# gk969/stm32-speech-recognition

Measured on AMD Instinct MI355X. Metric: utterances/sec (256-frame, 100 templates), higher is better.
Workload: dtype int32

## Files before the change

### stm32_speech_recognition_amd/csrc/k_mfcc.hip

```cpp
#include "sr_fft_dev.h"

#include <type_traits>

#ifndef SR_MEL_CHUNKED
#define SR_MEL_CHUNKED 1
#endif

namespace sr {

constexpr int kMfccWaves = 4;
constexpr int kFramesPerWave = 16, kFramesPerWaveMid = 4, kFramesPerWaveSmall = 1;
#ifndef SR_MAG_TAB_BINS
#define SR_MAG_TAB_BINS 8
#endif
constexpr int mfcc_tab_bins(int fpw) { return fpw == kFramesPerWave ? SR_MAG_TAB_BINS : 0; }
static_assert(SR_MAG_TAB_BINS == 0 || SR_MAG_TAB_BINS == 4 || SR_MAG_TAB_BINS == 8, "table bins per lane");
#ifndef SR_MFCC_PIPE
#define SR_MFCC_PIPE 1
#endif
#ifndef SR_MFCC_PIPE_PEEL
#define SR_MFCC_PIPE_PEEL 1
#endif
#ifndef SR_MFCC_PIPE_VMCNT
#define SR_MFCC_PIPE_VMCNT (SR_MFCC_PIPE_PEEL ? 3 : 0)
#endif
static_assert(SR_MFCC_PIPE_VMCNT == 0 || (SR_MFCC_PIPE_VMCNT == 3 && SR_MFCC_PIPE_PEEL), "younger loads counted by the wait");
constexpr bool mfcc_pipelined(int fpw) { return SR_MFCC_PIPE && mfcc_tab_bins(fpw) == 8; }
constexpr int kMelPad = kMel + 1;
__device__ __forceinline__ constexpr int mel_chunk_word(int j) { return 256 * ((j >> 2) & 1) + 4 * ((j >> 3) ^ (4 * ((j >> 2) & 1))) + (j & 3); }
constexpr int mfcc_wave_lds_words(int fpw) { return kXchgWords + fpw * kMelPad + 64; }

template <typename Base>
struct MfccTabArgs : Base {
    const uint16_t *mag_q;
    uint32_t mag_table_off;
};
template <typename Base>
constexpr int mfcc_feat_kind<MfccTabArgs<Base>> = mfcc_feat_kind<Base>;
template <typename Base>
static MfccTabArgs<Base> mfcc_tab_args(const Base &b, const MfccMagTab &tab)
{
    MfccTabArgs<Base> r;
    static_cast<Base &>(r) = b;
    r.mag_q = tab.mag_q;
    r.mag_table_off = tab.mag_table_off;
    return r;
}

template <int kFPW, typename Args = MfccTabArgs<MfccArgs>>
__global__ void __launch_bounds__(64 * kMfccWaves, 4) k_mfcc(const Args a)
{
    constexpr int kFeat = mfcc_feat_kind<Args>;
    constexpr uint32_t kFeatW = (kFeat == SR_FEAT_FFT || kFeat == SR_FEAT_MAG) ? kBins : kMel;
    constexpr int kWaveLdsWords = mfcc_wave_lds_words(kFPW);
    constexpr int kTabBins = mfcc_tab_bins(kFPW);
    constexpr bool kPipe = mfcc_pipelined(kFPW);
    extern __shared__ __attribute__((aligned(16))) uint32_t smem[];
    __shared__ uint32_t s_dctM[kCoef * kMelPad];
    __shared__ int s_dctS[kCoef * kMelPad];
    __shared__ u32x4 s_tw3[kTw3Row * 4], s_tw5[8 * 64];
    __shared__ u32x4 s_tm[4 * 64];
    const int lane = threadIdx.x & 63, w = __builtin_amdgcn_readfirstlane(threadIdx.x >> 6);
    uint32_t *buf = smem + w * kWaveLdsWords;
    uint32_t *xw = buf;
    uint32_t *powb = buf + kXchgWords, *moff = powb + kFPW * kMelPad;

    for (int i = threadIdx.x; i < kCoef * kMel; i += blockDim.x) {
        const int c = a.t.dct[i], o = (i / kMel) * kMelPad + i % kMel;
        s_dctM[o] = (uint32_t)(((c < 0 ? -c : c) * 262144 + 99) / 100);
        s_dctS[o] = (c > 0) - (c < 0);
    }
    __syncthreads();

    LaneTw tw;
    load_lane_tw(a.t, lane, tw);
    real_leg_tw(tw);
    if (w == 0 && lane < 4) {
        const uint32_t *f = &tw.s3[0][0][0];
#pragma unroll
        for (int c = 0; c < 8; c++) s_tw3[lane * kTw3Row + c] = u32x4{f[4 * c], f[4 * c + 1], f[4 * c + 2], f[4 * c + 3]};
    }
    if (w == 1 % kMfccWaves) store_tw32(s_tw5, lane, tw.s5);
#ifndef SR_INJECT_LDS_RACE
    if (w == 2 % kMfccWaves) {
#pragma unroll
        for (int c = 0; c < 2; c++) {
            s_tm[64 * c + lane] = *(const u32x4 *)(a.t.tri_even_m + 8 * lane + 4 * c);
            s_tm[64 * (c + 2) + lane] = *(const u32x4 *)(a.t.tri_odd_m + 8 * lane + 4 * c);
        }
    }
#endif
    __syncthreads();
#ifdef SR_INJECT_LDS_RACE
    if (w == 2 % kMfccWaves) {
#if SR_INJECT_LDS_RACE >= 2
        __builtin_amdgcn_s_sleep(127);
#endif
#pragma unroll
        for (int c = 0; c < 2; c++) {
            s_tm[64 * c + lane] = *(const u32x4 *)(a.t.tri_even_m + 8 * lane + 4 * c);
            s_tm[64 * (c + 2) + lane] = *(const u32x4 *)(a.t.tri_odd_m + 8 * lane + 4 * c);
        }
    }
#endif
    int hamm_m[3];
#pragma unroll
    for (int k = 0; k < 3; k++) hamm_m[k] = (lane + 64 * k < kFrameLen) ? hamm_fused_multiplier(a.t.hamm[lane + 64 * k]) : 0;
    int f_lo = 0, p_hi = 0, p_lo = 0, x_hi = 0, x_lo = 0;
    if (lane < kMel) {
        const int h = lane;
        f_lo = (h == 0) ? 0 : (int)a.t.tri_cen[h - 1];
        const int f_hi = (h == kMel - 1) ? kBins : (int)a.t.tri_cen[h + 1];
        const int ih = f_hi - 1, il = f_lo ? f_lo - 1 : 0, half = (h & 1) ? kBins : 0;
#if SR_MEL_CHUNKED
        p_hi = half + mel_chunk_word(ih), x_hi = (ih >> 3) > 0 ? (ih >> 3) - 1 : 0;
        p_lo = half + mel_chunk_word(il), x_lo = (il >> 3) > 0 ? (il >> 3) - 1 : 0;
#else
        p_hi = half + ih, x_hi = (ih >> 3) > 0 ? (ih >> 3) - 1 : 0;
        p_lo = half + il, x_lo = (il >> 3) > 0 ? (il >> 3) - 1 : 0;
#endif
    }
    const uint64_t mag_p = (uint64_t)a.mag_q;
    const u32x4 mag_rs = {(uint32_t)mag_p, (uint32_t)(mag_p >> 32) | (2u << 16), kMagTabEntries, 0x00027000u};
    const uint32_t tw_off = 32u * (uint32_t)lane;
#if SR_MEL_CHUNKED
    const int e_base = mel_chunk_word(lane);
    constexpr int kEs = 32, kEh = 128;
    const int c0 = mel_chunk_word(8 * lane), c1 = mel_chunk_word(8 * lane + 4);
#else
    const int e_base = lane;
    constexpr int kEs = 64, kEh = 256;
    const int c0 = 8 * lane, c1 = 8 * lane + 4;
#endif

    uint32_t item = blockIdx.x;
    uint32_t nx_nfrm = 0;
    int nx_mid = 0, nx_seg0 = 0;
    if (item < a.n_items) {
        const sr_vad_rec *rec = a.vad + item / a.tiles;
        nx_nfrm = rec->frm_num;
        nx_mid = (int)rec->atap.mid_val;
        nx_seg0 = rec->seg[0];
    }
    for (; item < a.n_items; item += gridDim.x) {
        const uint32_t b = item / a.tiles, tile = item - b * a.tiles;
        const uint32_t nfrm = nx_nfrm;
        const int mid = nx_mid, seg0 = nx_seg0;
        if (item + gridDim.x < a.n_items) {
            const sr_vad_rec *rec = a.vad + (item + gridDim.x) / a.tiles;
            nx_nfrm = rec->frm_num;
            nx_mid = (int)rec->atap.mid_val;
            nx_seg0 = rec->seg[0];
        }
        const uint16_t *row = a.pcm + (uint64_t)b * a.pcm_stride;
        int16_t *out = a.mfcc + (uint64_t)b * a.max_frames * kCoef;
        const uint32_t f0 = tile * (kMfccWaves * kFPW) + w * kFPW;
        uint32_t *frow = nullptr;
        if constexpr (kFeat != 0) frow = a.feat + (uint64_t)b * a.max_frames * kFeatW;
        uint32_t nf = 0;
        if (f0 < nfrm) nf = (nfrm - f0 < (uint32_t)kFPW) ? nfrm - f0 : (uint32_t)kFPW;

        uint32_t s_pp[3] = {0, 0, 0};
        if (nf) {
            const uint16_t *x = row + seg0 + (int)kHop * (int)f0;
#pragma unroll
            for (int k = 0; k < 3; k++) {
                const int i = lane + 64 * k;
                if (i < kFrameLen) s_pp[k] = *(const u32_align2 *)(x + i - 1);
            }
        }
        if constexpr (!kPipe)
        for (uint32_t fi = 0; fi < nf; fi++) {
#pragma unroll
            for (int k = 0; k < 3; k++) {
                const int i = lane + 64 * k;
                if (i < kFrameLen) k == 0 ? window_store<0>(xw, i, s_pp[k], mid, hamm_m[k]) : window_store<1>(xw, i, s_pp[k], mid, hamm_m[k]);
            }
            if (fi + 1 < nf) {
                const uint16_t *x = row + seg0 + (int)kHop * (int)(f0 + fi + 1);
#pragma unroll
                for (int k = 0; k < 3; k++) {
                    const int i = lane + 64 * k;
                    if (i < kFrameLen) s_pp[k] = *(const u32_align2 *)(x + i - 1);
                }
            }
            wave_sync();
            uint32_t v[4][4], u[4][4];
            fft_front_real160(xw, lane, tw, s_tw3, v);
            fft_exchange(buf, lane, v, u);
#pragma unroll
            for (int e4 = 0; e4 < 4; e4++) fft_pass4_dbl(u, e4, tw);
            wave_sync();
            uint32_t k5[4][4][2];
            load_tw32(s_tw5, lane, k5);
            uint32_t nn[8];
#pragma unroll
            for (int e3 = 0; e3 < 4; e3++) {
                bfly_pk_dbl<true, false, 0>(u[e3][0], u[e3][1], u[e3][2], u[e3][3], k5[e3][0][0], k5[e3][0][1], k5[e3][1][0],
                                            k5[e3][1][1], k5[e3][2][0], k5[e3][2][1], k5[e3][3][0], k5[e3][3][1]);
                if constexpr (kFeat == SR_FEAT_FFT) {
                    uint32_t *fr = frow + (f0 + fi) * kFeatW + lane + 64 * e3;
                    fr[0] = u[e3][0];
                    fr[256] = u[e3][1];
                }
                nn[2 * e3] = (uint32_t)sdot2z(u[e3][0], u[e3][0]);
                nn[2 * e3 + 1] = (uint32_t)sdot2z(u[e3][1], u[e3][1]);
            }
            const uint32_t nmax = max(max(max(max(nn[0], nn[1]), nn[2]), max(max(nn[3], nn[4]), nn[5])), max(nn[6], nn[7]));
#ifdef SR_TESTING
            const bool quiet = __builtin_expect(__builtin_amdgcn_ballot_w64(nmax > kMagSmallMax) == 0 && !a.mag_table_off, 1);
#else
            const bool quiet = __builtin_expect(__builtin_amdgcn_ballot_w64(nmax > kMagSmallMax) == 0, 1);
#endif
            u32x4 tw_e[2], tw_o[2];
            bool cheap = true;
            if (!quiet) {
#pragma unroll
                for (int c = 0; c < 2; c++) {
                    tw_e[c] = *(const u32x4 *)((const char *)a.t.tri_even32 + tw_off + 16 * c);
                    tw_o[c] = *(const u32x4 *)((const char *)a.t.tri_odd32 + tw_off + 16 * c);
                }
                cheap = __builtin_amdgcn_ballot_w64(nmax > a.mag_cheap_max) == 0;
            } else {
                asm volatile("" : "=v"(tw_e[0]), "=v"(tw_e[1]), "=v"(tw_o[0]), "=v"(tw_o[1]));
            }
            uint32_t *eb = buf + e_base;
            if (kTabBins > 0 && quiet) {
                uint32_t tq[8];
#pragma unroll
                for (int e3 = 0; e3 < 4; e3++) {
                    if constexpr (kTabBins == 8)
                        asm volatile("buffer_load_ushort %0, %1, %2, 0 idxen" : "=v"(tq[2 * e3]) : "v"(nn[2 * e3]), "s"(mag_rs));
                    asm volatile("buffer_load_ushort %0, %1, %2, 0 idxen" : "=v"(tq[2 * e3 + 1]) : "v"(nn[2 * e3 + 1]), "s"(mag_rs));
                }
                uint32_t q0s[4];
                if constexpr (kTabBins == 4) {
#pragma unroll
                    for (int e3 = 0; e3 < 4; e3++) q0s[e3] = cvt_u32(__builtin_amdgcn_sqrtf((float)(int)nn[2 * e3]) * 10.0f) << 2;
                }
                if constexpr (kTabBins == 8)
                    asm volatile("s_waitcnt vmcnt(0)" : "+v"(tq[0]), "+v"(tq[1]), "+v"(tq[2]), "+v"(tq[3]), "+v"(tq[4]), "+v"(tq[5]), "+v"(tq[6]), "+v"(tq[7]));
                else
                    asm volatile("s_waitcnt vmcnt(0)" : "+v"(tq[1]), "+v"(tq[3]), "+v"(tq[5]), "+v"(tq[7]));
#pragma unroll
                for (int e3 = 0; e3 < 4; e3++) {
                    uint32_t q0, q1 = tq[2 * e3 + 1];
                    if constexpr (kTabBins == 8) q0 = tq[2 * e3];
                    else q0 = q0s[e3];
                    if constexpr (kFeat == SR_FEAT_MAG) {
                        uint32_t *fr = frow + (f0 + fi) * kFeatW + lane + 64 * e3;
                        fr[0] = q0 >> 2;
                        fr[256] = q1 >> 2;
                    }
                    eb[kEs * e3] = umul24(q0, q0);
                    eb[kEs * e3 + kEh] = umul24(q1, q1);
                }
            } else if (cheap) {
#pragma unroll
                for (int e3 = 0; e3 < 4; e3++) {
                    const f32x2 m = f32x2{__builtin_amdgcn_sqrtf((float)(int)nn[2 * e3]), __builtin_amdgcn_sqrtf((float)(int)nn[2 * e3 + 1])} *
                                    f32x2{10.0f, 10.0f};
                    const uint32_t m0 = cvt_u32(m.x), m1 = cvt_u32(m.y);
                    if constexpr (kFeat == SR_FEAT_MAG) {
                        uint32_t *fr = frow + (f0 + fi) * kFeatW + lane + 64 * e3;
                        fr[0] = m0;
                        fr[256] = m1;
                    }
                    eb[kEs * e3] = umul24(m0, m0);
                    eb[kEs * e3 + kEh] = umul24(m1, m1);
                }
            } else {
#pragma unroll
                for (int e3 = 0; e3 < 4; e3++) {
                    const f32x2 m = sqrt_rn_int2(f32x2{(float)(int)nn[2 * e3], (float)(int)nn[2 * e3 + 1]}) * f32x2{10.0f, 10.0f};
                    const uint32_t m0 = cvt_u32(m.x), m1 = cvt_u32(m.y);
                    if constexpr (kFeat == SR_FEAT_MAG) {
                        uint32_t *fr = frow + (f0 + fi) * kFeatW + lane + 64 * e3;
                        fr[0] = m0;
                        fr[256] = m1;
                    }
                    eb[kEs * e3] = umul24(m0, m0);
                    eb[kEs * e3 + kEh] = umul24(m1, m1);
                }
            }
            wave_sync();
            uint32_t pe[8], po[8], xe, xo;
            {
                const uint4 q0 = *(const uint4 *)(buf + c0), q1 = *(const uint4 *)(buf + c1);
                const uint32_t e[8] = {q0.x, q0.y, q0.z, q0.w, q1.x, q1.y, q1.z, q1.w};
                uint32_t se = 0, so = 0;
                if (quiet) {
#pragma unroll
                    for (int c = 0; c < 2; c++) {
                        const u32x4 me = s_tm[64 * c + lane], mo = s_tm[64 * (c + 2) + lane];
#pragma unroll
                        for (int k = 0; k < 4; k++) {
                            const uint32_t es = kTabBins > 0 ? e[4 * c + k] : e[4 * c + k] << 4;
                            se += mel_term_fused(es, me[k]);
                            so += mel_term_fused(es, mo[k]);
                            pe[4 * c + k] = se;
                            po[4 * c + k] = so;
                        }
                    }
                } else {
#pragma unroll
                    for (int c = 0; c < 2; c++) {
#pragma unroll
                        for (int k = 0; k < 4; k++) {
                            se += e[4 * c + k] * tw_e[c][k] / 100u;
                            so += e[4 * c + k] * tw_o[c][k] / 100u;
                            pe[4 * c + k] = se;
                            po[4 * c + k] = so;
                        }
                    }
                }
                xe = wave_scan_incl(se);
                xo = wave_scan_incl(so);
            }
            *(uint4 *)(buf + c0) = make_uint4(pe[0], pe[1], pe[2], pe[3]);
            *(uint4 *)(buf + c1) = make_uint4(pe[4], pe[5], pe[6], pe[7]);
            *(uint4 *)(buf + kBins + c0) = make_uint4(po[0], po[1], po[2], po[3]);
            *(uint4 *)(buf + kBins + c1) = make_uint4(po[4], po[5], po[6], po[7]);
            buf[2 * kBins + lane] = xe;
            moff[lane] = xo;
            wave_sync();
            if (lane < kMel) {
                const uint32_t *X = (lane & 1) ? moff : buf + 2 * kBins;
                const uint32_t hi = buf[p_hi] + X[x_hi], lo = f_lo ? buf[p_lo] + X[x_lo] : 0u;
                powb[fi * kMelPad + lane] = hi - lo;
                if constexpr (kFeat == SR_FEAT_MEL) frow[(f0 + fi) * kFeatW + lane] = hi - lo;
            }
            wave_sync();
        } else {
            uint32_t mq[8] = {0, 0, 0, 0, 0, 0, 0, 0};
            bool pq = true;
            auto window = [&]() {
#pragma unroll
                for (int k = 0; k < 3; k++) {
                    const int i = lane + 64 * k;
                    if (i < kFrameLen) k == 0 ? window_store<0>(xw, i, s_pp[k], mid, hamm_m[k]) : window_store<1>(xw, i, s_pp[k], mid, hamm_m[k]);
                }
            };
            auto request = [&](uint32_t f) {
                const uint16_t *x = row + seg0 + (int)kHop * (int)(f0 + f);
#pragma unroll
                for (int k = 0; k < 3; k++) {
                    const int i = lane + 64 * k;
                    if (i < kFrameLen) s_pp[k] = *(const u32_align2 *)(x + i - 1);
                }
            };
            auto middle = [&](uint32_t fi, uint32_t (&v)[4][4], bool more) {
                uint32_t u[4][4];
                fft_exchange(buf, lane, v, u);
#pragma unroll
                for (int e4 = 0; e4 < 4; e4++) fft_pass4_dbl(u, e4, tw);
                wave_sync();
                uint32_t k5[4][4][2];
                load_tw32(s_tw5, lane, k5);
                uint32_t nn[8];
#pragma unroll
                for (int e3 = 0; e3 < 4; e3++) {
                    bfly_pk_dbl<true, false, 0>(u[e3][0], u[e3][1], u[e3][2], u[e3][3], k5[e3][0][0], k5[e3][0][1], k5[e3][1][0],
                                                k5[e3][1][1], k5[e3][2][0], k5[e3][2][1], k5[e3][3][0], k5[e3][3][1]);
                    if constexpr (kFeat == SR_FEAT_FFT) {
                        uint32_t *fr = frow + (f0 + fi) * kFeatW + lane + 64 * e3;
                        fr[0] = u[e3][0];
                        fr[256] = u[e3][1];
                    }
                    nn[2 * e3] = (uint32_t)sdot2z(u[e3][0], u[e3][0]);
                    nn[2 * e3 + 1] = (uint32_t)sdot2z(u[e3][1], u[e3][1]);
                }
                const uint32_t nmax = max(max(max(max(nn[0], nn[1]), nn[2]), max(max(nn[3], nn[4]), nn[5])), max(nn[6], nn[7]));
                if (more) {
                    wave_sync();
                    window();
                }
#ifdef SR_TESTING
                const bool quiet = __builtin_expect(__builtin_amdgcn_ballot_w64(nmax > kMagSmallMax) == 0 && !a.mag_table_off, 1);
#else
                const bool quiet = __builtin_expect(__builtin_amdgcn_ballot_w64(nmax > kMagSmallMax) == 0, 1);
#endif
                if (quiet) {
#pragma unroll
                    for (int k = 0; k < 8; k++) asm volatile("buffer_load_ushort %0, %1, %2, 0 idxen" : "=v"(mq[k]) : "v"(nn[k]), "s"(mag_rs));
                } else if (__builtin_amdgcn_ballot_w64(nmax > a.mag_cheap_max) == 0) {
#pragma unroll
                    for (int e3 = 0; e3 < 4; e3++) {
                        const f32x2 m = f32x2{__builtin_amdgcn_sqrtf((float)(int)nn[2 * e3]), __builtin_amdgcn_sqrtf((float)(int)nn[2 * e3 + 1])} *
                                        f32x2{10.0f, 10.0f};
                        mq[2 * e3] = cvt_u32(m.x);
                        mq[2 * e3 + 1] = cvt_u32(m.y);
                    }
                } else {
#pragma unroll
                    for (int e3 = 0; e3 < 4; e3++) {
                        const f32x2 m = sqrt_rn_int2(f32x2{(float)(int)nn[2 * e3], (float)(int)nn[2 * e3 + 1]}) * f32x2{10.0f, 10.0f};
                        mq[2 * e3] = cvt_u32(m.x);
                        mq[2 * e3 + 1] = cvt_u32(m.y);
                    }
                }
                pq = quiet;
                if (fi + 2 < nf) request(fi + 2);
            };
            auto back_end = [&](uint32_t r, auto young) {
                wave_sync();
                auto energies = [&]() {
                    uint32_t *eb = buf + e_base;
#pragma unroll
                    for (int e3 = 0; e3 < 4; e3++) {
                        const uint32_t q0 = mq[2 * e3], q1 = mq[2 * e3 + 1];
                        if constexpr (kFeat == SR_FEAT_MAG) {
                            uint32_t *fr = frow + (f0 + r) * kFeatW + lane + 64 * e3;
                            const uint32_t sh = pq ? 2u : 0u;
                            fr[0] = q0 >> sh;
                            fr[256] = q1 >> sh;
                        }
                        eb[kEs * e3] = umul24(q0, q0);
                        eb[kEs * e3 + kEh] = umul24(q1, q1);
                    }
                    wave_sync();
                };
                uint32_t pe[8], po[8], se = 0, so = 0;
                if (pq) {
                    if constexpr (decltype(young)::value)
                        asm volatile("s_waitcnt vmcnt(3)" : "+v"(mq[0]), "+v"(mq[1]), "+v"(mq[2]), "+v"(mq[3]), "+v"(mq[4]), "+v"(mq[5]), "+v"(mq[6]), "+v"(mq[7]));
                    else
                        asm volatile("s_waitcnt vmcnt(0)" : "+v"(mq[0]), "+v"(mq[1]), "+v"(mq[2]), "+v"(mq[3]), "+v"(mq[4]), "+v"(mq[5]), "+v"(mq[6]), "+v"(mq[7]));
                    energies();
                    const uint4 q0 = *(const uint4 *)(buf + c0), q1 = *(const uint4 *)(buf + c1);
                    const uint32_t e[8] = {q0.x, q0.y, q0.z, q0.w, q1.x, q1.y, q1.z, q1.w};
#pragma unroll
                    for (int c = 0; c < 2; c++) {
                        const u32x4 me = s_tm[64 * c + lane], mo = s_tm[64 * (c + 2) + lane];
#pragma unroll
                        for (int k = 0; k < 4; k++) {
                            se += mel_term_fused(e[4 * c + k], me[k]);
                            so += mel_term_fused(e[4 * c + k], mo[k]);
                            pe[4 * c + k] = se;
                            po[4 * c + k] = so;
                        }
                    }
                } else {
                    u32x4 tw_e[2], tw_o[2];
                    uint32_t off = tw_off;
                    asm("" : "+v"(off));
#pragma unroll
                    for (int c = 0; c < 2; c++) {
                        tw_e[c] = *(const u32x4 *)((const char *)a.t.tri_even32 + off + 16 * c);
                        tw_o[c] = *(const u32x4 *)((const char *)a.t.tri_odd32 + off + 16 * c);
                    }
                    energies();
                    const uint4 q0 = *(const uint4 *)(buf + c0), q1 = *(const uint4 *)(buf + c1);
                    const uint32_t e[8] = {q0.x, q0.y, q0.z, q0.w, q1.x, q1.y, q1.z, q1.w};
#pragma unroll
                    for (int c = 0; c < 2; c++) {
#pragma unroll
                        for (int k = 0; k < 4; k++) {
                            se += e[4 * c + k] * tw_e[c][k] / 100u;
                            so += e[4 * c + k] * tw_o[c][k] / 100u;
                            pe[4 * c + k] = se;
                            po[4 * c + k] = so;
                        }
                    }
                }
                const uint32_t xe = wave_scan_incl(se), xo = wave_scan_incl(so);
                *(uint4 *)(buf + c0) = make_uint4(pe[0], pe[1], pe[2], pe[3]);
                *(uint4 *)(buf + c1) = make_uint4(pe[4], pe[5], pe[6], pe[7]);
                *(uint4 *)(buf + kBins + c0) = make_uint4(po[0], po[1], po[2], po[3]);
                *(uint4 *)(buf + kBins + c1) = make_uint4(po[4], po[5], po[6], po[7]);
                buf[2 * kBins + lane] = xe;
                moff[lane] = xo;
                wave_sync();
                if (lane < kMel) {
                    const uint32_t *X = (lane & 1) ? moff : buf + 2 * kBins;
                    const uint32_t hi = buf[p_hi] + X[x_hi], lo = f_lo ? buf[p_lo] + X[x_lo] : 0u;
                    powb[r * kMelPad + lane] = hi - lo;
                    if constexpr (kFeat == SR_FEAT_MEL) frow[(f0 + r) * kFeatW + lane] = hi - lo;
                }
                wave_sync();
            };
            constexpr std::false_type kDrain{};
            if (nf) {
                window();
                if (nf > 1) request(1);
#if SR_MFCC_PIPE_PEEL
                constexpr std::integral_constant<bool, SR_MFCC_PIPE_VMCNT != 0> kSteady{};
                {
                    wave_sync();
                    uint32_t v[4][4];
                    fft_front_real160(xw, lane, tw, s_tw3, v);
                    middle(0, v, nf > 1);
                }
                for (uint32_t fi = 1; fi + 1 < nf; fi++) {
                    wave_sync();
                    uint32_t v[4][4];
                    fft_front_real160(xw, lane, tw, s_tw3, v);
                    back_end(fi - 1, kSteady);
                    middle(fi, v, true);
                }
                if (nf > 1) {
                    wave_sync();
                    uint32_t v[4][4];
                    fft_front_real160(xw, lane, tw, s_tw3, v);
                    back_end(nf - 2, kDrain);
                    middle(nf - 1, v, false);
                }
#else
                for (uint32_t fi = 0; fi < nf; fi++) {
                    wave_sync();
                    uint32_t v[4][4];
                    fft_front_real160(xw, lane, tw, s_tw3, v);
                    if (fi > 0) back_end(fi - 1, kDrain);
                    middle(fi, v, fi + 1 < nf);
                }
#endif
                back_end(nf - 1, kDrain);
            }
        }

        {
            constexpr int kLogRounds = (kFPW * kMelPad + 63) / 64;
            const uint32_t n_log = nf * kMelPad;
            uint32_t nv[kLogRounds], mv[kLogRounds];
            u32x2 tv[kLogRounds];
#pragma unroll
            for (int r = 0; r < kLogRounds; r++) {
                const uint32_t t = lane + 64u * r;
                nv[r] = powb[t];
                mv[r] = log100_est(nv[r]);
                tv[r] = *(const u32_pair_align4 *)((const char *)a.t.log_thr + 4u * mv[r]);
            }
#pragma unroll
            for (int r = 0; r < kLogRounds; r++) {
                const uint32_t t = lane + 64u * r;
                if (t < n_log) powb[t] = log100_fix(nv[r], mv[r], tv[r].x, tv[r].y) << 14;
            }
        }
        wave_sync();
        if constexpr (kFeat == SR_FEAT_LOGMEL) {
            uint32_t *fw = frow + f0 * kFeatW;
            for (uint32_t t = lane; t < nf * kFeatW; t += 64) {
                const uint32_t fi = t / kFeatW, h = t - fi * kFeatW;
                fw[t] = powb[fi * kMelPad + h] >> 14;
            }
        }
        {
            int16_t *out_w = out + (size_t)f0 * kCoef;
#pragma unroll
            for (uint32_t tl = lane; tl < (uint32_t)(kFPW * kCoef); tl += 64) {
                uint32_t t = tl;
                if constexpr (kPipe) asm volatile("" : "+v"(t));
                if (t < nf * kCoef) {
                    const uint32_t fi = umul24(t, 10923u) >> 17, h = t - umul24(fi, (uint32_t)kCoef);
                    const uint32_t *pw = powb + umul24(fi, (uint32_t)kMelPad), *dm = s_dctM + umul24(h, (uint32_t)kMelPad);
                    const int *ds = s_dctS + umul24(h, (uint32_t)kMelPad);
                    int acc = 0;
#pragma unroll
                    for (int i = 0; i < kMel; i++) acc = mad24((int)__umulhi(pw[i], dm[i]), ds[i], acc);
                    out_w[t] = (int16_t)acc;
                }
            }
        }
        wave_sync();
        {
            const uint32_t r0 = f0 + nf, r1 = (f0 + kFPW < a.max_frames) ? f0 + kFPW : a.max_frames;
            for (uint32_t t = r0 * kCoef + lane; t < r1 * kCoef && r0 < r1; t += 64) out[t] = 0;
        }
        if constexpr (kFeat != 0) {
            const uint32_t r0 = f0 + nf, r1 = (f0 + kFPW < a.max_frames) ? f0 + kFPW : a.max_frames;
            for (uint32_t t = r0 * kFeatW + lane; t < r1 * kFeatW && r0 < r1; t += 64) frow[t] = 0;
        }
    }
}

uint32_t mfcc_ext_frames_per_tile();
int mfcc_ext_occupancy(int *per_cu);
void launch_mfcc_ext(const MfccArgs &a, uint32_t grid, hipStream_t s);
void launch_mfcc_ext_features(const MfccArgs &a, int kind, uint32_t *feat, uint32_t grid, hipStream_t s);

uint32_t mfcc_frames_per_tile(uint32_t frame_len) { return frame_len == 320 ? mfcc_ext_frames_per_tile() : (uint32_t)(kMfccWaves * kFramesPerWave); }
uint32_t mfcc_frames_per_tile_small(uint32_t frame_len, uint32_t which)
{
    return frame_len == 320 ? mfcc_ext_frames_per_tile() : (uint32_t)(kMfccWaves * (which ? kFramesPerWaveSmall : kFramesPerWaveMid));
}

uint32_t mfcc_resident_workgroups(uint32_t frame_len)
{
    int dev = 0, n_cu = 0, per_cu = 0;
    if (hipGetDevice(&dev) != hipSuccess) return 0;
    if (hipDeviceGetAttribute(&n_cu, hipDeviceAttributeMultiprocessorCount, dev) != hipSuccess || n_cu < 1) return 0;
    int e;
    if (frame_len == 320)
        e = mfcc_ext_occupancy(&per_cu);
    else
        e = (int)hipOccupancyMaxActiveBlocksPerMultiprocessor(&per_cu, k_mfcc<kFramesPerWave>, 64 * kMfccWaves,
                                                              (size_t)kMfccWaves * mfcc_wave_lds_words(kFramesPerWave) * sizeof(uint32_t));
    if (e != (int)hipSuccess || per_cu < 1) return 0;
    return (uint32_t)(per_cu * n_cu);
}

void launch_mfcc(const MfccArgs &a, const MfccMagTab &tab, hipStream_t s)
{
    if (a.generic) {
        launch_mfcc_gen(a, s);
        return;
    }
    if (a.n_items == 0) return;
    const uint32_t cap = a.grid_cap ? a.grid_cap : 4096u;
    const uint32_t grid = a.n_items < cap ? a.n_items : cap;
    if (a.frame_len == 320) {
        launch_mfcc_ext(a, grid, s);
        return;
    }
    if (a.small_tiles == 2) {
        const size_t lds = (size_t)kMfccWaves * mfcc_wave_lds_words(kFramesPerWaveSmall) * sizeof(uint32_t);
        SR_LAUNCH_POINT(s, "k_mfcc");
        hipLaunchKernelGGL(k_mfcc<kFramesPerWaveSmall>, dim3(grid), dim3(64 * kMfccWaves), lds, s, mfcc_tab_args(a, tab));
        return;
    }
    if (a.small_tiles == 1) {
        const size_t lds = (size_t)kMfccWaves * mfcc_wave_lds_words(kFramesPerWaveMid) * sizeof(uint32_t);
        SR_LAUNCH_POINT(s, "k_mfcc");
        hipLaunchKernelGGL(k_mfcc<kFramesPerWaveMid>, dim3(grid), dim3(64 * kMfccWaves), lds, s, mfcc_tab_args(a, tab));
        return;
    }
    const size_t lds = (size_t)kMfccWaves * mfcc_wave_lds_words(kFramesPerWave) * sizeof(uint32_t);
    SR_LAUNCH_POINT(s, "k_mfcc");
    hipLaunchKernelGGL(k_mfcc<kFramesPerWave>, dim3(grid), dim3(64 * kMfccWaves), lds, s, mfcc_tab_args(a, tab));
}

template <int kFPW, int kKind>
static void launch_mfcc_feat_kind(const MfccArgs &a, const MfccMagTab &tab, uint32_t *feat, uint32_t grid, hipStream_t s)
{
    const size_t lds = (size_t)kMfccWaves * mfcc_wave_lds_words(kFPW) * sizeof(uint32_t);
    SR_LAUNCH_POINT(s, "k_mfcc");
    hipLaunchKernelGGL((k_mfcc<kFPW, MfccTabArgs<MfccFeatArgs<kKind>>>), dim3(grid), dim3(64 * kMfccWaves), lds, s,
                       mfcc_tab_args(mfcc_feat_args<kKind>(a, feat), tab));
}
template <int kFPW>
static void launch_mfcc_feat_form(const MfccArgs &a, const MfccMagTab &tab, int kind, uint32_t *feat, uint32_t grid, hipStream_t s)
{
    switch (kind) {
    case SR_FEAT_FFT: launch_mfcc_feat_kind<kFPW, SR_FEAT_FFT>(a, tab, feat, grid, s); break;
    case SR_FEAT_MAG: launch_mfcc_feat_kind<kFPW, SR_FEAT_MAG>(a, tab, feat, grid, s); break;
    case SR_FEAT_MEL: launch_mfcc_feat_kind<kFPW, SR_FEAT_MEL>(a, tab, feat, grid, s); break;
    case SR_FEAT_LOGMEL: launch_mfcc_feat_kind<kFPW, SR_FEAT_LOGMEL>(a, tab, feat, grid, s); break;
    default: break;
    }
}

void launch_mfcc_features(const MfccArgs &a, const MfccMagTab &tab, int kind, uint32_t *feat, hipStream_t s)
{
    if (a.generic) {
        launch_mfcc_gen_features(a, kind, feat, s);
        return;
    }
    if (a.n_items == 0) return;
    const uint32_t cap = a.grid_cap ? a.grid_cap : 4096u;
    const uint32_t grid = a.n_items < cap ? a.n_items : cap;
    if (a.frame_len == 320)
        launch_mfcc_ext_features(a, kind, feat, grid, s);
    else if (a.small_tiles == 2)
        launch_mfcc_feat_form<kFramesPerWaveSmall>(a, tab, kind, feat, grid, s);
    else if (a.small_tiles == 1)
        launch_mfcc_feat_form<kFramesPerWaveMid>(a, tab, kind, feat, grid, s);
    else
        launch_mfcc_feat_form<kFramesPerWave>(a, tab, kind, feat, grid, s);
}

}
```

Measured before the change: 3.379 million.

## Keep mel triangle weights in registers and store prefixes with addtid writes

In the pipelined MFCC path, each lane now loads its mel triangle weights into registers once, so the per-frame LDS reads of s_tm go away. The partial prefix sums are now written with sixteen ds_write_addtid_b32 instructions into a thread-id-strided layout, replacing four 128-bit vector stores into the chunk-swizzled layout. The mel gather indices are remapped to match the new layout. The change costs 16 extra VGPRs per lane and uses inline asm that sets m0, which may constrain occupancy and scheduling.

```diff
diff --git a/stm32_speech_recognition_amd/csrc/k_mfcc.hip b/stm32_speech_recognition_amd/csrc/k_mfcc.hip
--- a/stm32_speech_recognition_amd/csrc/k_mfcc.hip
+++ b/stm32_speech_recognition_amd/csrc/k_mfcc.hip
@@ -26,8 +26,47 @@
 #endif
 static_assert(SR_MFCC_PIPE_VMCNT == 0 || (SR_MFCC_PIPE_VMCNT == 3 && SR_MFCC_PIPE_PEEL), "younger loads counted by the wait");
 constexpr bool mfcc_pipelined(int fpw) { return SR_MFCC_PIPE && mfcc_tab_bins(fpw) == 8; }
+#ifndef SR_MFCC_TM_REGS
+#define SR_MFCC_TM_REGS 1
+#endif
+#ifdef SR_INJECT_LDS_RACE
+#undef SR_MFCC_TM_REGS
+#define SR_MFCC_TM_REGS 0
+#endif
+constexpr bool mfcc_tm_regs(int fpw) { return SR_MFCC_TM_REGS && mfcc_pipelined(fpw); }
 constexpr int kMelPad = kMel + 1;
 __device__ __forceinline__ constexpr int mel_chunk_word(int j) { return 256 * ((j >> 2) & 1) + 4 * ((j >> 3) ^ (4 * ((j >> 2) & 1))) + (j & 3); }
+#ifndef SR_MFCC_PREFIX_TID
+#define SR_MFCC_PREFIX_TID 1
+#endif
+__device__ __forceinline__ constexpr int mel_prefix_word(int j)
+{
+#if SR_MFCC_PREFIX_TID
+    return 64 * (j & 7) + (j >> 3);
+#elif SR_MEL_CHUNKED
+    return mel_chunk_word(j);
+#else
+    return j;
+#endif
+}
+#pragma clang diagnostic push
+#pragma clang diagnostic ignored "-Winline-asm"
+__device__ __forceinline__ void mel_prefix_store(uint32_t base, const uint32_t (&pe)[8], const uint32_t (&po)[8])
+{
+    static_assert(kBins == 512, "the offsets below are written out for two halves of 512 words");
+    asm volatile("s_mov_b32 m0, %16\n\ts_nop 0\n\t"
+                 "ds_write_addtid_b32 %0\n\tds_write_addtid_b32 %1 offset:256\n\tds_write_addtid_b32 %2 offset:512\n\t"
+                 "ds_write_addtid_b32 %3 offset:768\n\tds_write_addtid_b32 %4 offset:1024\n\tds_write_addtid_b32 %5 offset:1280\n\t"
+                 "ds_write_addtid_b32 %6 offset:1536\n\tds_write_addtid_b32 %7 offset:1792\n\t"
+                 "ds_write_addtid_b32 %8 offset:2048\n\tds_write_addtid_b32 %9 offset:2304\n\tds_write_addtid_b32 %10 offset:2560\n\t"
+                 "ds_write_addtid_b32 %11 offset:2816\n\tds_write_addtid_b32 %12 offset:3072\n\tds_write_addtid_b32 %13 offset:3328\n\t"
+                 "ds_write_addtid_b32 %14 offset:3584\n\tds_write_addtid_b32 %15 offset:3840"
+                 :
+                 : "v"(pe[0]), "v"(pe[1]), "v"(pe[2]), "v"(pe[3]), "v"(pe[4]), "v"(pe[5]), "v"(pe[6]), "v"(pe[7]), "v"(po[0]),
+                   "v"(po[1]), "v"(po[2]), "v"(po[3]), "v"(po[4]), "v"(po[5]), "v"(po[6]), "v"(po[7]), "s"(base)
+                 : "m0", "memory");
+}
+#pragma clang diagnostic pop
 constexpr int mfcc_wave_lds_words(int fpw) { return kXchgWords + fpw * kMelPad + 64; }
 
 template <typename Base>
@@ -55,6 +94,7 @@
     constexpr int kWaveLdsWords = mfcc_wave_lds_words(kFPW);
     constexpr int kTabBins = mfcc_tab_bins(kFPW);
     constexpr bool kPipe = mfcc_pipelined(kFPW);
+    constexpr bool kTmRegs = mfcc_tm_regs(kFPW);
     extern __shared__ __attribute__((aligned(16))) uint32_t smem[];
     __shared__ uint32_t s_dctM[kCoef * kMelPad];
     __shared__ int s_dctS[kCoef * kMelPad];
@@ -64,6 +104,8 @@
     uint32_t *buf = smem + w * kWaveLdsWords;
     uint32_t *xw = buf;
     uint32_t *powb = buf + kXchgWords, *moff = powb + kFPW * kMelPad;
+    const uint32_t buf_lds = (uint32_t)(uintptr_t)(const __attribute__((address_space(3))) uint32_t *)buf;
+    (void)buf_lds;
 
     for (int i = threadIdx.x; i < kCoef * kMel; i += blockDim.x) {
         const int c = a.t.dct[i], o = (i / kMel) * kMelPad + i % kMel;
@@ -81,8 +123,16 @@
         for (int c = 0; c < 8; c++) s_tw3[lane * kTw3Row + c] = u32x4{f[4 * c], f[4 * c + 1], f[4 * c + 2], f[4 * c + 3]};
     }
     if (w == 1 % kMfccWaves) store_tw32(s_tw5, lane, tw.s5);
+    u32x4 tm_r[4];
+    if constexpr (kTmRegs) {
+#pragma unroll
+        for (int c = 0; c < 2; c++) {
+            tm_r[c] = *(const u32x4 *)(a.t.tri_even_m + 8 * lane + 4 * c);
+            tm_r[c + 2] = *(const u32x4 *)(a.t.tri_odd_m + 8 * lane + 4 * c);
+        }
+    }
 #ifndef SR_INJECT_LDS_RACE
-    if (w == 2 % kMfccWaves) {
+    if (!kTmRegs && w == 2 % kMfccWaves) {
 #pragma unroll
         for (int c = 0; c < 2; c++) {
             s_tm[64 * c + lane] = *(const u32x4 *)(a.t.tri_even_m + 8 * lane + 4 * c);
@@ -112,13 +162,8 @@
         f_lo = (h == 0) ? 0 : (int)a.t.tri_cen[h - 1];
         const int f_hi = (h == kMel - 1) ? kBins : (int)a.t.tri_cen[h + 1];
         const int ih = f_hi - 1, il = f_lo ? f_lo - 1 : 0, half = (h & 1) ? kBins : 0;
-#if SR_MEL_CHUNKED
-        p_hi = half + mel_chunk_word(ih), x_hi = (ih >> 3) > 0 ? (ih >> 3) - 1 : 0;
-        p_lo = half + mel_chunk_word(il), x_lo = (il >> 3) > 0 ? (il >> 3) - 1 : 0;
-#else
-        p_hi = half + ih, x_hi = (ih >> 3) > 0 ? (ih >> 3) - 1 : 0;
-        p_lo = half + il, x_lo = (il >> 3) > 0 ? (il >> 3) - 1 : 0;
-#endif
+        p_hi = half + mel_prefix_word(ih), x_hi = (ih >> 3) > 0 ? (ih >> 3) - 1 : 0;
+        p_lo = half + mel_prefix_word(il), x_lo = (il >> 3) > 0 ? (il >> 3) - 1 : 0;
     }
     const uint64_t mag_p = (uint64_t)a.mag_q;
     const u32x4 mag_rs = {(uint32_t)mag_p, (uint32_t)(mag_p >> 32) | (2u << 16), kMagTabEntries, 0x00027000u};
@@ -169,6 +214,16 @@
                 if (i < kFrameLen) s_pp[k] = *(const u32_align2 *)(x + i - 1);
             }
         }
+        auto store_prefixes = [&](const uint32_t (&pe)[8], const uint32_t (&po)[8]) {
+#if SR_MFCC_PREFIX_TID
+            mel_prefix_store(buf_lds, pe, po);
+#else
+            *(uint4 *)(buf + c0) = make_uint4(pe[0], pe[1], pe[2], pe[3]);
+            *(uint4 *)(buf + c1) = make_uint4(pe[4], pe[5], pe[6], pe[7]);
+            *(uint4 *)(buf + kBins + c0) = make_uint4(po[0], po[1], po[2], po[3]);
+            *(uint4 *)(buf + kBins + c1) = make_uint4(po[4], po[5], po[6], po[7]);
+#endif
+        };
         if constexpr (!kPipe)
         for (uint32_t fi = 0; fi < nf; fi++) {
 #pragma unroll
@@ -317,10 +372,7 @@
                 xe = wave_scan_incl(se);
                 xo = wave_scan_incl(so);
             }
-            *(uint4 *)(buf + c0) = make_uint4(pe[0], pe[1], pe[2], pe[3]);
-            *(uint4 *)(buf + c1) = make_uint4(pe[4], pe[5], pe[6], pe[7]);
-            *(uint4 *)(buf + kBins + c0) = make_uint4(po[0], po[1], po[2], po[3]);
-            *(uint4 *)(buf + kBins + c1) = make_uint4(po[4], po[5], po[6], po[7]);
+            store_prefixes(pe, po);
             buf[2 * kBins + lane] = xe;
             moff[lane] = xo;
             wave_sync();
@@ -431,7 +483,9 @@
                     const uint32_t e[8] = {q0.x, q0.y, q0.z, q0.w, q1.x, q1.y, q1.z, q1.w};
 #pragma unroll
                     for (int c = 0; c < 2; c++) {
-                        const u32x4 me = s_tm[64 * c + lane], mo = s_tm[64 * (c + 2) + lane];
+                        u32x4 me, mo;
+                        if constexpr (kTmRegs) me = tm_r[c], mo = tm_r[c + 2];
+                        else me = s_tm[64 * c + lane], mo = s_tm[64 * (c + 2) + lane];
 #pragma unroll
                         for (int k = 0; k < 4; k++) {
                             se += mel_term_fused(e[4 * c + k], me[k]);
@@ -464,10 +518,7 @@
                     }
                 }
                 const uint32_t xe = wave_scan_incl(se), xo = wave_scan_incl(so);
-                *(uint4 *)(buf + c0) = make_uint4(pe[0], pe[1], pe[2], pe[3]);
-                *(uint4 *)(buf + c1) = make_uint4(pe[4], pe[5], pe[6], pe[7]);
-                *(uint4 *)(buf + kBins + c0) = make_uint4(po[0], po[1], po[2], po[3]);
-                *(uint4 *)(buf + kBins + c1) = make_uint4(po[4], po[5], po[6], po[7]);
+                store_prefixes(pe, po);
                 buf[2 * kBins + lane] = xe;
                 moff[lane] = xo;
                 wave_sync();
```

New measurement: 3.446 million (median of 6 runs). +2.0%, better.
